# yisol/IDM-VTON

Hardware: NVIDIA H100
Metric: try-on images/sec @768x1024, 30 steps, CFG 2.0 (higher is better)
Workload: dtype fp16

## Files before the change

idm-vton_b200/csrc/gemm.cu:

```cuda
#include "gemm_common.cuh"
#include "host.h"
#include "wgmma.cuh"

namespace vton {

enum : int { KIND_F16 = 0, KIND_F16IN_F32OUT = 1, KIND_TF32 = 2, KIND_E4M3 = 3 };

template <int BN, int STAGES>
struct SmemLayout {
  static constexpr int B_BYTES = BN * 128;
  static constexpr int STAGE_BYTES = A_BYTES + B_BYTES;
  static constexpr int BAR_OFFSET = STAGES * STAGE_BYTES;
  static constexpr int TOTAL = BAR_OFFSET + 256 + 1024;
};

constexpr int GEMM_THREADS = 384;
constexpr int GEMM_PRODUCER_REGS = 40;
constexpr int GEMM_CONSUMER_REGS = 232;

template <int BN>
constexpr int E4M3_SUB = BN == 256 ? 64 : (BN == 192 ? 96 : BN);

template <int BN, int STAGES, bool GEGLU, bool SC, int KIND>
__global__ void __launch_bounds__(GEMM_THREADS, 1)
gemm_conv_kernel(const __grid_constant__ CUtensorMap tmA, const __grid_constant__ CUtensorMap tmB,
                 const __grid_constant__ CUtensorMap tmS0, const __grid_constant__ CUtensorMap tmS1,
                 const __grid_constant__ CUtensorMap tmBs, const GemmParams p) {
  using L = SmemLayout<BN, STAGES>;
  constexpr int KBK = KIND == KIND_TF32 ? 32 : (KIND == KIND_E4M3 ? 128 : 64);
  constexpr bool F16_EPI = KIND == KIND_F16 || KIND == KIND_E4M3;
  extern __shared__ uint8_t smem_raw[];
  const uint32_t smem_base = (smem_u32(smem_raw) + 1023u) & ~1023u;
  const uint32_t bar_base = smem_base + L::BAR_OFFSET;
  auto full_bar = [&](int s) { return bar_base + 8u * s; };
  auto empty_bar = [&](int s) { return bar_base + 8u * (STAGES + s); };

  const int warp = threadIdx.x >> 5;
  const int lane = threadIdx.x & 31;
  const int total_slabs = p.slabs_main + (SC ? p.slabs_sc : 0);

  if (warp == 8 && lane == 0) {
    tma_prefetch_desc(&tmA);
    tma_prefetch_desc(&tmB);
    if (SC) {
      tma_prefetch_desc(&tmS0);
      tma_prefetch_desc(&tmS1);
      tma_prefetch_desc(&tmBs);
    }
    for (int s = 0; s < STAGES; ++s) {
      mbar_init(full_bar(s), 1);
      mbar_init(empty_bar(s), 2);
    }
    fence_barrier_init();
  }
  pdl_wait();
  __syncthreads();
  pdl_launch_dependents();

  if (warp >= 8) {
    setmaxnreg_dec<GEMM_PRODUCER_REGS>();
    if (warp == 8 && lane == 0) {
      uint32_t it = 0;
      for (int tile = blockIdx.x; tile < p.total_tiles; tile += gridDim.x) {
        const int n0 = (tile % p.n_tiles) * BN;
        const int m_tile = tile / p.n_tiles;
        int b0 = 0, y0 = 0, x0 = 0;
        if (p.conv) {
          x0 = (m_tile % p.tiles_x) * p.bw;
          y0 = ((m_tile / p.tiles_x) % p.tiles_y) * p.bh;
          b0 = (m_tile / (p.tiles_x * p.tiles_y)) * p.bb;
        }
        for (int s = 0; s < total_slabs; ++s, ++it) {
          const int stage = it % STAGES;
          const uint32_t phase = (it / STAGES) & 1;
          mbar_wait(empty_bar(stage), phase ^ 1);
          const uint32_t a_dst = smem_base + stage * L::STAGE_BYTES;
          const uint32_t b_dst = a_dst + A_BYTES;
          mbar_expect_tx(full_bar(stage), L::STAGE_BYTES);
          if (s < p.slabs_main) {
            if (p.conv) {
              const int tap = s / p.cin_slabs;
              const int c0 = (s - tap * p.cin_slabs) * KBK;
              const int dy = tap / 3 - 1, dx = tap % 3 - 1;
              tma_load_4d(a_dst, &tmA, full_bar(stage), c0, x0 * p.stride + dx, y0 * p.stride + dy, b0);
              tma_load_2d(b_dst, &tmB, full_bar(stage), c0, tap * p.cout + n0);
            } else {
              tma_load_2d(a_dst, &tmA, full_bar(stage), s * KBK, m_tile * BM);
              tma_load_2d(b_dst, &tmB, full_bar(stage), s * KBK, n0);
            }
          } else {
            const int ss = s - p.slabs_main;
            if (ss < p.sc_split)
              tma_load_4d(a_dst, &tmS0, full_bar(stage), ss * BK, x0, y0, b0);
            else
              tma_load_4d(a_dst, &tmS1, full_bar(stage), (ss - p.sc_split) * BK, x0, y0, b0);
            tma_load_2d(b_dst, &tmBs, full_bar(stage), ss * BK, n0);
          }
        }
      }
    }
    return;
  }

  setmaxnreg_inc<GEMM_CONSUMER_REGS>();
  const int wg = warp >> 2;
  const int r_local = wg * 64 + ((warp & 3) << 4) + (lane >> 2);
  float acc[BN / 2];
  float acc_sc[BN / 2];
  uint32_t it = 0;
  auto release = [&](uint32_t slab) {
    if ((threadIdx.x & 127) == 0) mbar_arrive(empty_bar(slab % STAGES));
  };
  auto run_slabs = [&](float (&accr)[BN / 2], int s_begin, int s_end) {
    for (int s = s_begin; s < s_end; ++s, ++it) {
      const int stage = it % STAGES;
      mbar_wait(full_bar(stage), (it / STAGES) & 1);
      const uint32_t a_src = smem_base + stage * L::STAGE_BYTES + wg * (64 * 128);
      const uint32_t b_src = smem_base + stage * L::STAGE_BYTES + A_BYTES;
      wgmma_fence();
#pragma unroll
      for (int k = 0; k < 4; ++k) {
        const uint64_t da = make_gmma_desc_sw128(a_src + k * 32, 0, 1024);
        const uint64_t db = make_gmma_desc_sw128(b_src + k * 32, 0, 1024);
        const int scale_d = (s > s_begin || k > 0) ? 1 : 0;
        if constexpr (KIND == KIND_TF32) {
          WgmmaTF32SS<BN>::mma(accr, da, db, scale_d);
        } else {
          WgmmaF16SS<BN, 0>::mma(accr, da, db, scale_d);
        }
      }
      wgmma_commit();
      wgmma_wait<1>();
      if (s > 0) release(it - 1);
    }
  };
  auto run_slabs_promoted = [&](float (&accr)[BN / 2], int s_begin, int s_end) {
    constexpr int SUB = E4M3_SUB<BN>;
    for (int s = s_begin; s < s_end; ++s, ++it) {
      const int stage = it % STAGES;
      mbar_wait(full_bar(stage), (it / STAGES) & 1);
      const uint32_t a_src = smem_base + stage * L::STAGE_BYTES + wg * (64 * 128);
      const uint32_t b_src = smem_base + stage * L::STAGE_BYTES + A_BYTES;
#pragma unroll
      for (int sub = 0; sub < BN / SUB; ++sub) {
        float part[SUB / 2];
        wgmma_fence();
#pragma unroll
        for (int k = 0; k < 4; ++k) {
          const uint64_t da = make_gmma_desc_sw128(a_src + k * 32, 0, 1024);
          const uint64_t db = make_gmma_desc_sw128(b_src + sub * SUB * 128 + k * 32, 0, 1024);
          WgmmaE4M3SS<SUB>::mma(part, da, db, k > 0 ? 1 : 0);
        }
        wgmma_commit();
        wgmma_wait<0>();
        fence_regs(part);
#pragma unroll
        for (int j = 0; j < SUB / 2; ++j) accr[sub * (SUB / 2) + j] = s > s_begin ? accr[sub * (SUB / 2) + j] + part[j] : part[j];
      }
      release(it);
    }
  };
  for (int tile = blockIdx.x; tile < p.total_tiles; tile += gridDim.x) {
    EpilogueF16<BN, GEGLU, SC, KIND == KIND_E4M3> epi;
    if constexpr (F16_EPI) epi.begin(p, tile / p.n_tiles, tile % p.n_tiles, r_local);
    if constexpr (KIND == KIND_E4M3) {
      run_slabs_promoted(acc, 0, p.slabs_main);
    } else {
      run_slabs(acc, 0, p.slabs_main);
      if constexpr (SC) run_slabs(acc_sc, p.slabs_main, total_slabs);
      wgmma_wait<0>();
      fence_regs(acc);
      if (SC) fence_regs(acc_sc);
      release(it - 1);
    }
    if constexpr (F16_EPI) {
      epi.finish(p, acc, acc_sc);
    } else {
      epilogue_f32<BN>(p, tile / p.n_tiles, tile % p.n_tiles, r_local, acc);
    }
  }
}

template <int BN, int STAGES, bool GEGLU, bool SC, int KIND>
static int launch_variant(const CUtensorMap& tmA, const CUtensorMap& tmB, const CUtensorMap& tmS0,
                          const CUtensorMap& tmS1, const CUtensorMap& tmBs, const GemmParams& p, cudaStream_t stream) {
  using L = SmemLayout<BN, STAGES>;
  static_assert(L::TOTAL <= 227 * 1024, "shared memory budget");
  auto kern = gemm_conv_kernel<BN, STAGES, GEGLU, SC, KIND>;
  static bool configured = false;
  if (!configured) {
    VTON_CUDA(cudaFuncSetAttribute(kern, cudaFuncAttributeMaxDynamicSharedMemorySize, L::TOTAL));
    configured = true;
  }
  const int grid = p.total_tiles < num_sms() ? p.total_tiles : num_sms();
  VTON_CUDA(launch_kernel(kern, dim3(grid), dim3(GEMM_THREADS), L::TOTAL, stream, tmA, tmB, tmS0, tmS1, tmBs, p));
  count_launch();
  return kOk;
}

void set_auto_v2(int) {}
void set_cluster4(int) {}

static int pick_bn(int N, int m_tiles, bool geglu, bool has_shortcut, int force_bn) {
  if (force_bn >= 2000) force_bn -= 2000;
  else if (force_bn >= 1000) force_bn -= 1000;
  auto usable = [&](int bn) {
    if (geglu && ((bn != 256 && bn != 128) || N % bn != 0)) return false;
    if (has_shortcut && bn > 128) return false;
    return true;
  };
  if (force_bn) {
    const bool known = force_bn == 64 || force_bn == 128 || force_bn == 160 || force_bn == 192 || force_bn == 256;
    return known && usable(force_bn) ? force_bn : 0;
  }
  const int sms = num_sms();
  const int cands[5] = {256, 192, 160, 128, 64};
  double best = 1e300;
  int best_bn = 0;
  for (int bn : cands) {
    if (!usable(bn)) continue;
    if (bn != 128 && N % bn != 0 && !(bn == 64 && N < 64)) continue;
    const long long tiles = static_cast<long long>(m_tiles) * cdiv(N, bn);
    const long long waves = (tiles + sms - 1) / sms;
    const double cost = static_cast<double>(waves) * (bn + 64);
    if (cost < best * 0.999) {
      best = cost;
      best_bn = bn;
    }
  }
  return best_bn ? best_bn : 128;
}

template <int KIND>
static int dispatch(int bn, bool geglu, const CUtensorMap& tmA, const CUtensorMap& tmB, const CUtensorMap& tmS0,
                    const CUtensorMap& tmS1, const CUtensorMap& tmBs, GemmParams& p, int m_tiles,
                    cudaStream_t stream) {
  p.n_tiles = cdiv(p.N, bn);
  p.total_tiles = m_tiles * p.n_tiles;
  if (geglu) {
    if (bn == 128) return launch_variant<128, 6, true, false, KIND>(tmA, tmB, tmS0, tmS1, tmBs, p, stream);
    if (bn == 256) return launch_variant<256, 4, true, false, KIND>(tmA, tmB, tmS0, tmS1, tmBs, p, stream);
    set_last_error("GEGLU epilogue supports BN 128/256 only (got %d)", bn);
    return kErrUnsupported;
  }
  if constexpr (KIND == KIND_F16) {
    if (p.slabs_sc) {
      if (bn == 64) return launch_variant<64, 8, false, true, KIND_F16>(tmA, tmB, tmS0, tmS1, tmBs, p, stream);
      if (bn == 128) return launch_variant<128, 6, false, true, KIND_F16>(tmA, tmB, tmS0, tmS1, tmBs, p, stream);
      set_last_error("shortcut epilogue supports BN 64/128 only (got %d)", bn);
      return kErrUnsupported;
    }
  }
  switch (bn) {
    case 64: return launch_variant<64, 8, false, false, KIND>(tmA, tmB, tmS0, tmS1, tmBs, p, stream);
    case 128: return launch_variant<128, 6, false, false, KIND>(tmA, tmB, tmS0, tmS1, tmBs, p, stream);
    case 160: return launch_variant<160, 5, false, false, KIND>(tmA, tmB, tmS0, tmS1, tmBs, p, stream);
    case 192: return launch_variant<192, 4, false, false, KIND>(tmA, tmB, tmS0, tmS1, tmBs, p, stream);
    case 256: return launch_variant<256, 4, false, false, KIND>(tmA, tmB, tmS0, tmS1, tmBs, p, stream);
  }
  set_last_error("unsupported BN %d", bn);
  return kErrUnsupported;
}

int gemm_f16_impl(const void* A, long long lda, const void* W, long long ldw, void* out, long long ldo, int M, int N,
                  int K, const void* bias, const void* residual, long long ldr, const void* rowvec, long long ld_rowvec,
                  int rows_per_sample, int flags, int force_bn, cudaStream_t stream) {
  const int geglu = flags & 1;
  VTON_CHECK_ARG(M > 0 && N > 0 && K > 0, "gemm: empty problem M=%d N=%d K=%d", M, N, K);
  VTON_CHECK_ARG(K % 64 == 0, "gemm: K=%d must be a multiple of 64", K);
  VTON_CHECK_ARG(N % 8 == 0 && lda % 8 == 0 && ldw % 8 == 0 && ldo % 8 == 0, "gemm: N/lda/ldw/ldo must be multiples of 8");
  VTON_CHECK_ARG(!geglu || (N % 16 == 0 && !residual && !rowvec), "gemm: bad GEGLU configuration");
  VTON_CHECK_ARG(aligned_to(out, 16) && aligned_to(bias, 16) && aligned_to(residual, 16) && aligned_to(rowvec, 16),
                 "gemm: out/bias/residual/rowvec must be 16-byte aligned");
  VTON_CHECK_ARG((!residual || ldr % 8 == 0) && (!rowvec || ld_rowvec % 8 == 0),
                 "gemm: ldr=%lld / ld_rowvec=%lld must be multiples of 8", ldr, ld_rowvec);
  const int bn = pick_bn(N, cdiv(M, BM), geglu != 0, false, force_bn);
  VTON_CHECK_ARG(bn != 0, "gemm: tile width force_bn=%d unsupported for this problem (N=%d, geglu=%d)", force_bn, N, geglu);
  VTON_CHECK_ARG(!geglu || N % bn == 0, "gemm: GEGLU needs N %% BN == 0 (N=%d, BN=%d)", N, bn);
  CUtensorMap tmA, tmB;
  {
    uint64_t dims[2] = {static_cast<uint64_t>(K), static_cast<uint64_t>(M)};
    uint64_t strides[1] = {static_cast<uint64_t>(lda) * 2};
    uint32_t box[2] = {64, 128};
    if (int e = encode_tmap_f16(&tmA, A, 2, dims, strides, box)) return e;
  }
  {
    uint64_t dims[2] = {static_cast<uint64_t>(K), static_cast<uint64_t>(N)};
    uint64_t strides[1] = {static_cast<uint64_t>(ldw) * 2};
    uint32_t box[2] = {64, static_cast<uint32_t>(bn)};
    if (int e = encode_tmap_f16(&tmB, W, 2, dims, strides, box)) return e;
  }
  GemmParams p{};
  p.out = static_cast<__half*>(out);
  p.ld_out = static_cast<int>(ldo);
  p.M = M;
  p.N = N;
  p.bias = static_cast<const __half*>(bias);
  p.residual = static_cast<const __half*>(residual);
  p.ld_res = static_cast<int>(ldr);
  p.rowvec = static_cast<const __half*>(rowvec);
  p.ld_rowvec = static_cast<int>(ld_rowvec);
  p.rows_per_sample = rows_per_sample;
  p.slabs_main = K / 64;
  p.act_gelu = (flags & 4) ? 2 : ((flags & 2) ? 1 : 0);
  return dispatch<KIND_F16>(bn, geglu != 0, tmA, tmB, tmA, tmA, tmB, p, cdiv(M, BM), stream);
}

int gemm_e4m3_impl(const void* A, long long lda, const void* a_scale, const void* W, long long ldw, const void* w_scale,
                   void* out, long long ldo, int M, int N, int K, const void* bias, const void* residual, long long ldr,
                   int flags, int force_bn, cudaStream_t stream) {
  const int geglu = flags & 1;
  VTON_CHECK_ARG(M > 0 && N > 0 && K > 0, "gemm_e4m3: empty problem M=%d N=%d K=%d", M, N, K);
  VTON_CHECK_ARG(K % 128 == 0, "gemm_e4m3: K=%d must be a multiple of 128", K);
  VTON_CHECK_ARG((flags & ~1) == 0, "gemm_e4m3: flags=%d unsupported (only GEGLU = 1)", flags);
  VTON_CHECK_ARG(A && W && out && a_scale && w_scale, "gemm_e4m3: A, W, out, a_scale and w_scale must not be null");
  VTON_CHECK_ARG(lda % 16 == 0 && ldw % 16 == 0, "gemm_e4m3: lda=%lld / ldw=%lld must be multiples of 16 bytes", lda, ldw);
  VTON_CHECK_ARG(N % 8 == 0 && ldo % 8 == 0, "gemm_e4m3: N/ldo must be multiples of 8");
  VTON_CHECK_ARG(!geglu || (N % 16 == 0 && !residual), "gemm_e4m3: bad GEGLU configuration");
  VTON_CHECK_ARG(aligned_to(A, 16) && aligned_to(W, 16) && aligned_to(out, 16) && aligned_to(bias, 16) &&
                     aligned_to(residual, 16) && aligned_to(a_scale, 4) && aligned_to(w_scale, 8),
                 "gemm_e4m3: A/W/out/bias/residual must be 16-byte aligned, a_scale 4-byte, w_scale 8-byte");
  VTON_CHECK_ARG(!residual || ldr % 8 == 0, "gemm_e4m3: ldr=%lld must be a multiple of 8", ldr);
  const int bn = pick_bn(N, cdiv(M, BM), geglu != 0, false, force_bn);
  VTON_CHECK_ARG(bn != 0, "gemm_e4m3: tile width force_bn=%d unsupported for this problem (N=%d, geglu=%d)", force_bn, N,
                 geglu);
  VTON_CHECK_ARG(!geglu || N % bn == 0, "gemm_e4m3: GEGLU needs N %% BN == 0 (N=%d, BN=%d)", N, bn);
  CUtensorMap tmA, tmB;
  {
    uint64_t dims[2] = {static_cast<uint64_t>(K), static_cast<uint64_t>(M)};
    uint64_t strides[1] = {static_cast<uint64_t>(lda)};
    uint32_t box[2] = {128, 128};
    if (int e = encode_tmap_u8(&tmA, A, 2, dims, strides, box)) return e;
  }
  {
    uint64_t dims[2] = {static_cast<uint64_t>(K), static_cast<uint64_t>(N)};
    uint64_t strides[1] = {static_cast<uint64_t>(ldw)};
    uint32_t box[2] = {128, static_cast<uint32_t>(bn)};
    if (int e = encode_tmap_u8(&tmB, W, 2, dims, strides, box)) return e;
  }
  GemmParams p{};
  p.out = static_cast<__half*>(out);
  p.ld_out = static_cast<int>(ldo);
  p.M = M;
  p.N = N;
  p.bias = static_cast<const __half*>(bias);
  p.residual = static_cast<const __half*>(residual);
  p.ld_res = static_cast<int>(ldr);
  p.slabs_main = K / 128;
  p.a_scale = static_cast<const float*>(a_scale);
  p.w_scale = static_cast<const float*>(w_scale);
  return dispatch<KIND_E4M3>(bn, geglu != 0, tmA, tmB, tmA, tmA, tmB, p, cdiv(M, BM), stream);
}

static void pick_box(int B, int H, int W, int* bw, int* bh, int* bb) {
  int w = 1;
  while (w < 128 && W % (w * 2) == 0) w *= 2;
  int h = 1;
  while (w * h < 128 && h * 2 <= H) h *= 2;
  *bw = w;
  *bh = h;
  *bb = 128 / (w * h);
  (void)B;
}

static int encode_nhwc(CUtensorMap* tm, const void* base, int B, int H, int W, int C, int ldc, int bw, int bh, int bb,
                       int pixel_step = 1) {
  uint64_t dims[4] = {static_cast<uint64_t>(C), static_cast<uint64_t>(W), static_cast<uint64_t>(H),
                      static_cast<uint64_t>(B)};
  uint64_t strides[3] = {static_cast<uint64_t>(ldc) * 2, static_cast<uint64_t>(W) * ldc * 2,
                         static_cast<uint64_t>(H) * W * ldc * 2};
  uint32_t box[4] = {64, static_cast<uint32_t>(bw * pixel_step), static_cast<uint32_t>(bh * pixel_step),
                     static_cast<uint32_t>(bb)};
  uint32_t estr[4] = {1, static_cast<uint32_t>(pixel_step), static_cast<uint32_t>(pixel_step), 1};
  return encode_tmap_f16(tm, base, 4, dims, strides, box, pixel_step > 1 ? estr : nullptr);
}

int conv3x3_impl(const void* x, long long ldx, int B, int Hin, int Win, int Cin, const void* w, int Cout, const void* bias,
                 const void* temb, long long ld_temb, const void* sc0, int C0, const void* sc1, int C1, const void* w_sc,
                 const void* bias_sc, const void* residual, long long ldr, void* out, long long ldo, int force_bn,
                 int stride, cudaStream_t stream) {
  VTON_CHECK_ARG(B > 0 && Hin > 0 && Win > 0, "conv3x3: empty input");
  VTON_CHECK_ARG(stride == 1 || stride == 2, "conv3x3: stride %d unsupported", stride);
  VTON_CHECK_ARG(stride == 1 || (!w_sc && !residual), "conv3x3: stride 2 has no shortcut / residual form");
  const int H = (Hin - 1) / stride + 1, W = (Win - 1) / stride + 1;
  VTON_CHECK_ARG(Cin % 64 == 0, "conv3x3: Cin=%d must be a multiple of 64 (pad channels)", Cin);
  VTON_CHECK_ARG(Cout % 8 == 0 && ldo % 8 == 0 && ldx % 8 == 0, "conv3x3: Cout/ldo/ldx must be multiples of 8");
  VTON_CHECK_ARG(C0 % 64 == 0 && C1 % 64 == 0, "conv3x3: shortcut source channels must be multiples of 64");
  VTON_CHECK_ARG(!(w_sc && residual), "conv3x3: shortcut conv and identity residual are exclusive");
  VTON_CHECK_ARG(aligned_to(out, 16) && aligned_to(bias, 16) && aligned_to(temb, 16) && aligned_to(bias_sc, 16) &&
                     aligned_to(residual, 16),
                 "conv3x3: out/bias/temb/bias_sc/residual must be 16-byte aligned");
  VTON_CHECK_ARG((!residual || ldr % 8 == 0) && (!temb || ld_temb % 8 == 0),
                 "conv3x3: ldr=%lld / ld_temb=%lld must be multiples of 8", ldr, ld_temb);
  int bw, bh, bb;
  pick_box(B, H, W, &bw, &bh, &bb);
  const int m_tiles_est = (W / bw) * cdiv(H, bh) * cdiv(B, bb);
  const int bn = pick_bn(Cout, m_tiles_est, false, w_sc != nullptr, force_bn);
  VTON_CHECK_ARG(bn != 0, "conv3x3: tile width force_bn=%d unsupported (a fused shortcut takes 64 or 128)", force_bn);
  CUtensorMap tmA, tmB, tmS0, tmS1, tmBs;
  VTON_CHECK_ARG(stride == 1 || (bw * 2 <= 256 && bh * 2 <= 256), "conv3x3: stride-2 box too large");
  if (int e = encode_nhwc(&tmA, x, B, Hin, Win, Cin, static_cast<int>(ldx), bw, bh, bb, stride)) return e;
  {
    uint64_t dims[2] = {static_cast<uint64_t>(Cin), static_cast<uint64_t>(9) * Cout};
    uint64_t strides[1] = {static_cast<uint64_t>(Cin) * 2};
    uint32_t box[2] = {64, static_cast<uint32_t>(bn)};
    if (int e = encode_tmap_f16(&tmB, w, 2, dims, strides, box)) return e;
  }
  tmS0 = tmA;
  tmS1 = tmA;
  tmBs = tmB;
  GemmParams p{};
  if (w_sc) {
    VTON_CHECK_ARG(sc0 && C0 > 0, "conv3x3: shortcut needs a source");
    if (int e = encode_nhwc(&tmS0, sc0, B, H, W, C0, C0, bw, bh, bb)) return e;
    if (sc1 && C1 > 0) {
      if (int e = encode_nhwc(&tmS1, sc1, B, H, W, C1, C1, bw, bh, bb)) return e;
    }
    const int Csc = C0 + (sc1 ? C1 : 0);
    uint64_t dims[2] = {static_cast<uint64_t>(Csc), static_cast<uint64_t>(Cout)};
    uint64_t strides[1] = {static_cast<uint64_t>(Csc) * 2};
    uint32_t box[2] = {64, static_cast<uint32_t>(bn)};
    if (int e = encode_tmap_f16(&tmBs, w_sc, 2, dims, strides, box)) return e;
    p.slabs_sc = Csc / 64;
    p.sc_split = C0 / 64;
  }
  p.out = static_cast<__half*>(out);
  p.ld_out = static_cast<int>(ldo);
  p.M = B * H * W;
  p.N = Cout;
  p.bias = static_cast<const __half*>(bias);
  p.bias_sc = static_cast<const __half*>(bias_sc);
  p.residual = static_cast<const __half*>(residual);
  p.ld_res = static_cast<int>(ldr);
  p.rowvec = static_cast<const __half*>(temb);
  p.ld_rowvec = static_cast<int>(ld_temb);
  p.slabs_main = 9 * (Cin / 64);
  p.conv = 1;
  p.stride = stride;
  p.H = H;
  p.W = W;
  p.B = B;
  p.bw = bw;
  p.bh = bh;
  p.bb = bb;
  p.tiles_x = W / bw;
  p.tiles_y = cdiv(H, bh);
  p.cin_slabs = Cin / 64;
  p.cout = Cout;
  const int m_tiles = p.tiles_x * p.tiles_y * cdiv(B, bb);
  return dispatch<KIND_F16>(bn, false, tmA, tmB, tmS0, tmS1, tmBs, p, m_tiles, stream);
}

int conv3x3_f32_impl(const void* x, int B, int H, int W, int Cin, const void* w, int Cout, const void* bias,
                     const void* residual, void* out, int in_fp16, cudaStream_t stream) {
  VTON_CHECK_ARG(B > 0 && H > 0 && W > 0, "conv3x3_f32: empty input");
  VTON_CHECK_ARG(Cin % 32 == 0 && Cout % 32 == 0 && Cout >= 64, "conv3x3_f32: Cin=%d / Cout=%d must be multiples of 32 (Cout >= 64)", Cin, Cout);
  VTON_CHECK_ARG(!in_fp16 || Cin % 64 == 0, "conv3x3_f32: fp16 operands need Cin=%d to be a multiple of 64", Cin);
  VTON_CHECK_ARG(x && w && out, "conv3x3_f32: null pointer");
  const int esz = in_fp16 ? 2 : 4;
  const int bk = in_fp16 ? 64 : 32;
  int bw, bh, bb;
  pick_box(B, H, W, &bw, &bh, &bb);
  VTON_CHECK_ARG(bw * bh * bb == 128 && bw >= 8, "conv3x3_f32: W=%d H=%d cannot be tiled into 128-pixel boxes", W, H);
  const int m_tiles = (W / bw) * cdiv(H, bh) * cdiv(B, bb);
  const int bn = pick_bn(Cout, m_tiles, false, false, Cout % 256 == 0 ? 256 : 128);
  CUtensorMap tmA, tmB;
  {
    uint64_t dims[4] = {static_cast<uint64_t>(Cin), static_cast<uint64_t>(W), static_cast<uint64_t>(H), static_cast<uint64_t>(B)};
    uint64_t strides[3] = {static_cast<uint64_t>(Cin) * esz, static_cast<uint64_t>(W) * Cin * esz,
                           static_cast<uint64_t>(H) * W * Cin * esz};
    uint32_t box[4] = {static_cast<uint32_t>(bk), static_cast<uint32_t>(bw), static_cast<uint32_t>(bh), static_cast<uint32_t>(bb)};
    if (int e = in_fp16 ? encode_tmap_f16(&tmA, x, 4, dims, strides, box) : encode_tmap_f32(&tmA, x, 4, dims, strides, box)) return e;
  }
  {
    uint64_t dims[2] = {static_cast<uint64_t>(Cin), static_cast<uint64_t>(9) * Cout};
    uint64_t strides[1] = {static_cast<uint64_t>(Cin) * esz};
    uint32_t box[2] = {static_cast<uint32_t>(bk), static_cast<uint32_t>(bn)};
    if (int e = in_fp16 ? encode_tmap_f16(&tmB, w, 2, dims, strides, box) : encode_tmap_f32(&tmB, w, 2, dims, strides, box)) return e;
  }
  GemmParams p{};
  p.out_f32 = static_cast<float*>(out);
  p.bias_f32 = static_cast<const float*>(bias);
  p.res_f32 = static_cast<const float*>(residual);
  p.M = B * H * W;
  p.N = Cout;
  p.slabs_main = 9 * (Cin / bk);
  p.conv = 1;
  p.stride = 1;
  p.H = H;
  p.W = W;
  p.B = B;
  p.bw = bw;
  p.bh = bh;
  p.bb = bb;
  p.tiles_x = W / bw;
  p.tiles_y = cdiv(H, bh);
  p.cin_slabs = Cin / bk;
  p.cout = Cout;
  p.n_tiles = cdiv(Cout, bn);
  p.total_tiles = m_tiles * p.n_tiles;
  if (in_fp16) {
    if (bn == 256) return launch_variant<256, 4, false, false, KIND_F16IN_F32OUT>(tmA, tmB, tmA, tmA, tmB, p, stream);
    return launch_variant<128, 6, false, false, KIND_F16IN_F32OUT>(tmA, tmB, tmA, tmA, tmB, p, stream);
  }
  if (bn == 256) return launch_variant<256, 4, false, false, KIND_TF32>(tmA, tmB, tmA, tmA, tmB, p, stream);
  return launch_variant<128, 6, false, false, KIND_TF32>(tmA, tmB, tmA, tmA, tmB, p, stream);
}

}
```

idm-vton_b200/csrc/gemm_common.cuh:

```cuda
#pragma once
#include "common.cuh"

namespace vton {

struct GemmParams {
  __half* out;
  int ld_out;
  int M, N;
  const __half* bias;
  const __half* bias_sc;
  const __half* residual;
  int ld_res;
  const __half* rowvec;
  int ld_rowvec;
  int rows_per_sample;
  int slabs_main;
  int slabs_sc;
  int sc_split;
  int conv;
  int H, W, B;
  int bw, bh, bb;
  int tiles_x, tiles_y;
  int cin_slabs;
  int cout;
  int n_tiles;
  int total_tiles;
  int act_gelu;
  int stride;
  float* out_f32;
  const float* bias_f32;
  const float* res_f32;
  const float* a_scale;
  const float* w_scale;
};

constexpr int BM = 128;
constexpr int BK = 64;
constexpr int A_BYTES = BM * BK * 2;

__device__ __forceinline__ void map_row(const GemmParams& p, int m_tile, int r_local, long long* out_row, int* sample) {
  *out_row = -1;
  if (p.conv) {
    const int tx = m_tile % p.tiles_x;
    const int ty = (m_tile / p.tiles_x) % p.tiles_y;
    const int tb = m_tile / (p.tiles_x * p.tiles_y);
    const int lx = r_local % p.bw;
    const int ly = (r_local / p.bw) % p.bh;
    const int lb = r_local / (p.bw * p.bh);
    const int b = tb * p.bb + lb, y = ty * p.bh + ly, x = tx * p.bw + lx;
    if (b < p.B && y < p.H && x < p.W) *out_row = (static_cast<long long>(b) * p.H + y) * p.W + x;
    *sample = b;
  } else {
    const int m = m_tile * BM + r_local;
    if (m < p.M) *out_row = m;
    *sample = p.rows_per_sample > 0 ? m / p.rows_per_sample : 0;
  }
}

__device__ __forceinline__ float gelu_erf_fast(float x) {
  const float ax = fabsf(x) * 0.70710678118654752f;
  const float t = __fdividef(1.0f, fmaf(0.3275911f, ax, 1.0f));
  float poly = fmaf(t, 1.061405429f, -1.453152027f);
  poly = fmaf(poly, t, 1.421413741f);
  poly = fmaf(poly, t, -0.284496736f);
  poly = fmaf(poly, t, 0.254829592f);
  poly *= t;
  float e;
  const float arg = -ax * ax * 1.4426950408889634f;
  asm("ex2.approx.ftz.f32 %0, %1;" : "=f"(e) : "f"(arg));
  const float erf_abs = fmaf(-poly, e, 1.0f);
  const float erf_v = copysignf(erf_abs, x);
  return 0.5f * x * (1.0f + erf_v);
}

__device__ __forceinline__ void quad_transpose(uint32_t (&w)[4], int q) {
  {
    const bool odd = (q & 1) != 0;
    const uint32_t s0 = __shfl_xor_sync(0xffffffffu, odd ? w[0] : w[1], 1);
    const uint32_t s1 = __shfl_xor_sync(0xffffffffu, odd ? w[2] : w[3], 1);
    if (odd) w[0] = s0, w[2] = s1;
    else w[1] = s0, w[3] = s1;
  }
  {
    const bool hi = (q & 2) != 0;
    const uint32_t s0 = __shfl_xor_sync(0xffffffffu, hi ? w[0] : w[2], 2);
    const uint32_t s1 = __shfl_xor_sync(0xffffffffu, hi ? w[1] : w[3], 2);
    if (hi) w[0] = s0, w[1] = s1;
    else w[2] = s0, w[3] = s1;
  }
}

__device__ __forceinline__ float2 ldg_h2(const __half* src) {
  return unpack_h2(__ldg(reinterpret_cast<const uint32_t*>(src)));
}

template <int BN, bool GEGLU, bool SC, bool SCALED = false>
struct EpilogueF16 {
  static constexpr int OUT_COLS = GEGLU ? BN / 2 : BN;
  static constexpr int CHUNKS = OUT_COLS / 32;
  static constexpr bool HAS_RES = !GEGLU && !SC;
  static constexpr int RES_AHEAD = (!HAS_RES || SCALED) ? 1 : (CHUNKS < 4 ? CHUNKS : 4);

  int q, n0, out_n0, out_N;
  long long out_row[2];
  int sample[2];
  uint32_t bias[BN / 8];
  uint32_t bias_sc[SC ? BN / 8 : 1];
  uint4 res[2][RES_AHEAD];
  float a_scale[SCALED ? 2 : 1];

  __device__ __forceinline__ int own_col(int c) const { return out_n0 + (4 * c + q) * 8; }

  __device__ __forceinline__ void load_res(const GemmParams& p, int c) {
#pragma unroll
    for (int h = 0; h < 2; ++h) {
      uint4 u = make_uint4(0u, 0u, 0u, 0u);
      if (p.residual && out_row[h] >= 0 && own_col(c) < out_N)
        u = *reinterpret_cast<const uint4*>(p.residual + out_row[h] * p.ld_res + own_col(c));
      res[h][c % RES_AHEAD] = u;
    }
  }

  __device__ __forceinline__ void begin(const GemmParams& p, int m_tile, int n_tile, int r_local) {
    q = threadIdx.x & 3;
    n0 = n_tile * BN;
    out_n0 = GEGLU ? n_tile * (BN / 2) : n0;
    out_N = GEGLU ? p.N / 2 : p.N;
#pragma unroll
    for (int h = 0; h < 2; ++h) map_row(p, m_tile, r_local + 8 * h, &out_row[h], &sample[h]);
    if constexpr (SCALED) {
#pragma unroll
      for (int h = 0; h < 2; ++h) a_scale[h] = out_row[h] >= 0 ? __ldg(p.a_scale + out_row[h]) : 0.0f;
    }
#pragma unroll
    for (int i = 0; i < BN / 8; ++i) {
      const bool ok = n0 + i * 8 < p.N;
      bias[i] = (p.bias && ok) ? __ldg(reinterpret_cast<const uint32_t*>(p.bias + n0 + i * 8 + 2 * q)) : 0u;
      if (SC) bias_sc[i] = (p.bias_sc && ok) ? __ldg(reinterpret_cast<const uint32_t*>(p.bias_sc + n0 + i * 8 + 2 * q)) : 0u;
    }
    if (HAS_RES) {
#pragma unroll
      for (int c = 0; c < RES_AHEAD; ++c) load_res(p, c);
    }
  }

  __device__ __forceinline__ void finish(const GemmParams& p, const float (&acc)[BN / 2], const float (&acc_sc)[BN / 2]) {
    const __half* rowvec_row[2];
#pragma unroll
    for (int h = 0; h < 2; ++h)
      rowvec_row[h] = (p.rowvec && out_row[h] >= 0) ? p.rowvec + static_cast<long long>(sample[h]) * p.ld_rowvec : nullptr;
#pragma unroll
    for (int c = 0; c < CHUNKS; ++c) {
      if (out_n0 + c * 32 >= out_N) break;
#pragma unroll
      for (int h = 0; h < 2; ++h) {
        uint32_t w[4];
#pragma unroll
        for (int g = 0; g < 4; ++g) {
          const int i = 4 * c + g;
          const bool col_ok = out_n0 + i * 8 < out_N;
          float v0 = acc[4 * i + 2 * h], v1 = acc[4 * i + 2 * h + 1];
          float2 w_scale[GEGLU ? 2 : 1];
          if constexpr (SCALED) {
#pragma unroll
            for (int e = 0; e < (GEGLU ? 2 : 1); ++e) {
              const int col = n0 + (i + e * (BN / 16)) * 8 + 2 * q;
              w_scale[e] = col < p.N ? __ldg(reinterpret_cast<const float2*>(p.w_scale + col)) : make_float2(0.f, 0.f);
            }
            v0 = __fmul_rn(__fmul_rn(v0, a_scale[h]), w_scale[0].x);
            v1 = __fmul_rn(__fmul_rn(v1, a_scale[h]), w_scale[0].y);
          }
          if (GEGLU) {
            float g0 = acc[4 * (i + BN / 16) + 2 * h], g1 = acc[4 * (i + BN / 16) + 2 * h + 1];
            if constexpr (SCALED) {
              g0 = __fmul_rn(__fmul_rn(g0, a_scale[h]), w_scale[GEGLU ? 1 : 0].x);
              g1 = __fmul_rn(__fmul_rn(g1, a_scale[h]), w_scale[GEGLU ? 1 : 0].y);
            }
            if (p.bias && col_ok) {
              const float2 b = unpack_h2(bias[i]), bg = unpack_h2(bias[i + BN / 16]);
              v0 += b.x, v1 += b.y, g0 += bg.x, g1 += bg.y;
            }
            v0 = round_h(v0) * round_h(gelu_erf_fast(round_h(g0)));
            v1 = round_h(v1) * round_h(gelu_erf_fast(round_h(g1)));
          } else {
            if (p.bias && col_ok) {
              const float2 b = unpack_h2(bias[i]);
              v0 += b.x, v1 += b.y;
            }
            if (p.act_gelu) {
              const float x0 = round_h(v0), x1 = round_h(v1);
              v0 = p.act_gelu == 2 ? __fdividef(x0, 1.0f + __expf(-1.702f * x0)) : gelu_erf_fast(x0);
              v1 = p.act_gelu == 2 ? __fdividef(x1, 1.0f + __expf(-1.702f * x1)) : gelu_erf_fast(x1);
            }
            if (rowvec_row[h] != nullptr && col_ok) {
              const float2 t = ldg_h2(rowvec_row[h] + n0 + i * 8 + 2 * q);
              v0 = round_h(v0) + t.x, v1 = round_h(v1) + t.y;
            }
            if (SC) {
              float s0 = acc_sc[4 * i + 2 * h], s1 = acc_sc[4 * i + 2 * h + 1];
              if (p.bias_sc && col_ok) {
                const float2 b = unpack_h2(bias_sc[i]);
                s0 += b.x, s1 += b.y;
              }
              v0 = round_h(s0) + round_h(v0), v1 = round_h(s1) + round_h(v1);
            }
          }
          w[g] = pack_h2(v0, v1);
        }
        quad_transpose(w, q);
        if (out_row[h] < 0 || own_col(c) >= out_N) continue;
        if (HAS_RES && p.residual) {
          const uint4 u = res[h][c % RES_AHEAD];
          const uint32_t r[4] = {u.x, u.y, u.z, u.w};
#pragma unroll
          for (int j = 0; j < 4; ++j) {
            const float2 a = unpack_h2(w[j]), d = unpack_h2(r[j]);
            w[j] = pack_h2(a.x + d.x, a.y + d.y);
          }
        }
        *reinterpret_cast<uint4*>(p.out + out_row[h] * p.ld_out + own_col(c)) = make_uint4(w[0], w[1], w[2], w[3]);
      }
      if (HAS_RES && c + RES_AHEAD < CHUNKS) load_res(p, c + RES_AHEAD);
    }
  }
};

template <int BN>
__device__ __forceinline__ void epilogue_f32(const GemmParams& p, int m_tile, int n_tile, int r_local,
                                             const float (&acc)[BN / 2]) {
  const int q = threadIdx.x & 3;
  const int n0 = n_tile * BN;
  long long out_row[2];
#pragma unroll
  for (int h = 0; h < 2; ++h) {
    int sample;
    map_row(p, m_tile, r_local + 8 * h, &out_row[h], &sample);
  }
#pragma unroll
  for (int i = 0; i < BN / 8; ++i) {
    if (n0 + i * 8 >= p.N) break;
    const int ncol = n0 + i * 8 + 2 * q;
    float2 b = make_float2(0.0f, 0.0f);
    if (p.bias_f32 != nullptr) b = __ldg(reinterpret_cast<const float2*>(p.bias_f32 + ncol));
#pragma unroll
    for (int h = 0; h < 2; ++h) {
      if (out_row[h] < 0) continue;
      float2 v = make_float2(acc[4 * i + 2 * h], acc[4 * i + 2 * h + 1]);
      if (p.bias_f32 != nullptr) v.x += b.x, v.y += b.y;
      if (p.res_f32 != nullptr) {
        const float2 r = __ldg(reinterpret_cast<const float2*>(p.res_f32 + out_row[h] * p.N + ncol));
        v.x += r.x, v.y += r.y;
      }
      *reinterpret_cast<float2*>(p.out_f32 + out_row[h] * p.N + ncol) = v;
    }
  }
}

}
```

Measured before the change: 0.8340.

## Stage GEMM epilogue through shared memory with dedicated store warps

Consumer warpgroups now write finished fp16 tiles into a shared-memory staging buffer instead of storing directly to global memory. Three idle producer-side warps prefetch residual rows with bulk async copies into that buffer and then perform the global stores, synchronised through new mbarriers, so stores overlap the next tile's mainloop. It also specialises the epilogue on activation and rowvec flags, rebalances register limits, and cuts BN=256 stages from 4 to 3 to fit the staging buffer. This adds synchronisation, and the single staging buffer can stall consumers until the store warps finish.

```diff
diff --git a/idm-vton_b200/csrc/gemm.cu b/idm-vton_b200/csrc/gemm.cu
--- a/idm-vton_b200/csrc/gemm.cu
+++ b/idm-vton_b200/csrc/gemm.cu
@@ -6,17 +6,22 @@
 
 enum : int { KIND_F16 = 0, KIND_F16IN_F32OUT = 1, KIND_TF32 = 2, KIND_E4M3 = 3 };
 
-template <int BN, int STAGES>
+constexpr bool f16_out(int kind) { return kind == KIND_F16 || kind == KIND_E4M3; }
+
+template <int BN, int STAGES, bool GEGLU, int KIND>
 struct SmemLayout {
   static constexpr int B_BYTES = BN * 128;
   static constexpr int STAGE_BYTES = A_BYTES + B_BYTES;
-  static constexpr int BAR_OFFSET = STAGES * STAGE_BYTES;
-  static constexpr int TOTAL = BAR_OFFSET + 256 + 1024;
+  static constexpr int STAGING_OFFSET = STAGES * STAGE_BYTES;
+  static constexpr int STAGING_BYTES = f16_out(KIND) ? StagingTile<BN, GEGLU>::BYTES : 0;
+  static constexpr int BAR_OFFSET = STAGING_OFFSET + STAGING_BYTES;
+  static constexpr int ROWS_OFFSET = BAR_OFFSET + 256;
+  static constexpr int TOTAL = ROWS_OFFSET + (f16_out(KIND) ? 2 * BM * 4 : 0) + 1024;
 };
 
 constexpr int GEMM_THREADS = 384;
-constexpr int GEMM_PRODUCER_REGS = 40;
-constexpr int GEMM_CONSUMER_REGS = 232;
+constexpr int GEMM_PRODUCER_REGS = 56;
+constexpr int GEMM_CONSUMER_REGS = 224;
 
 template <int BN>
 constexpr int E4M3_SUB = BN == 256 ? 64 : (BN == 192 ? 96 : BN);
@@ -26,20 +31,23 @@
 gemm_conv_kernel(const __grid_constant__ CUtensorMap tmA, const __grid_constant__ CUtensorMap tmB,
                  const __grid_constant__ CUtensorMap tmS0, const __grid_constant__ CUtensorMap tmS1,
                  const __grid_constant__ CUtensorMap tmBs, const GemmParams p) {
-  using L = SmemLayout<BN, STAGES>;
+  using L = SmemLayout<BN, STAGES, GEGLU, KIND>;
   constexpr int KBK = KIND == KIND_TF32 ? 32 : (KIND == KIND_E4M3 ? 128 : 64);
-  constexpr bool F16_EPI = KIND == KIND_F16 || KIND == KIND_E4M3;
+  constexpr bool F16_EPI = f16_out(KIND);
   extern __shared__ uint8_t smem_raw[];
   const uint32_t smem_base = (smem_u32(smem_raw) + 1023u) & ~1023u;
   const uint32_t bar_base = smem_base + L::BAR_OFFSET;
   auto full_bar = [&](int s) { return bar_base + 8u * s; };
   auto empty_bar = [&](int s) { return bar_base + 8u * (STAGES + s); };
+  const uint32_t staged_bar = bar_base + 8u * (2 * STAGES);
+  const uint32_t ready_bar = bar_base + 8u * (2 * STAGES + 1);
+  const uint32_t staging = smem_base + L::STAGING_OFFSET;
+  auto staging_ptr = [&]() { return smem_raw + (smem_base - smem_u32(smem_raw)) + L::STAGING_OFFSET; };
+  auto row_table = [&]() { return reinterpret_cast<int*>(smem_raw + (smem_base - smem_u32(smem_raw)) + L::ROWS_OFFSET); };
 
   const int warp = threadIdx.x >> 5;
-  const int lane = threadIdx.x & 31;
-  const int total_slabs = p.slabs_main + (SC ? p.slabs_sc : 0);
-
-  if (warp == 8 && lane == 0) {
+
+  if (threadIdx.x == 8 * 32) {
     tma_prefetch_desc(&tmA);
     tma_prefetch_desc(&tmB);
     if (SC) {
@@ -51,6 +59,10 @@
       mbar_init(full_bar(s), 1);
       mbar_init(empty_bar(s), 2);
     }
+    if (F16_EPI) {
+      mbar_init(staged_bar, 256);
+      mbar_init(ready_bar, EpilogueStore<BN, GEGLU>::THREADS);
+    }
     fence_barrier_init();
   }
   pdl_wait();
@@ -59,7 +71,8 @@
 
   if (warp >= 8) {
     setmaxnreg_dec<GEMM_PRODUCER_REGS>();
-    if (warp == 8 && lane == 0) {
+    if (threadIdx.x == 8 * 32) {
+      const int total_slabs = p.slabs_main + (SC ? p.slabs_sc : 0);
       uint32_t it = 0;
       for (int tile = blockIdx.x; tile < p.total_tiles; tile += gridDim.x) {
         const int n0 = (tile % p.n_tiles) * BN;
@@ -98,12 +111,15 @@
           }
         }
       }
+    } else if (F16_EPI && warp > 8) {
+      EpilogueStore<BN, GEGLU>::run(p, staging, staging_ptr(), row_table(), staged_bar, ready_bar, threadIdx.x - 9 * 32);
     }
     return;
   }
 
   setmaxnreg_inc<GEMM_CONSUMER_REGS>();
   const int wg = warp >> 2;
+  const int lane = threadIdx.x & 31;
   const int r_local = wg * 64 + ((warp & 3) << 4) + (lane >> 2);
   float acc[BN / 2];
   float acc_sc[BN / 2];
@@ -167,14 +183,20 @@
       run_slabs_promoted(acc, 0, p.slabs_main);
     } else {
       run_slabs(acc, 0, p.slabs_main);
-      if constexpr (SC) run_slabs(acc_sc, p.slabs_main, total_slabs);
+      if constexpr (SC) run_slabs(acc_sc, p.slabs_main, p.slabs_main + p.slabs_sc);
       wgmma_wait<0>();
       fence_regs(acc);
       if (SC) fence_regs(acc_sc);
       release(it - 1);
     }
     if constexpr (F16_EPI) {
-      epi.finish(p, acc, acc_sc);
+      mbar_wait(ready_bar, ((tile - blockIdx.x) / gridDim.x) & 1);
+      if (!GEGLU && p.act_gelu) epi.template stage<true, true>(p, acc, acc_sc, r_local, staging);
+      else if (!GEGLU && p.rowvec) epi.template stage<false, true>(p, acc, acc_sc, r_local, staging);
+      else epi.template stage<false, false>(p, acc, acc_sc, r_local, staging);
+      mbar_arrive(staged_bar);
+      if (tile + static_cast<int>(gridDim.x) >= p.total_tiles)
+        EpilogueStore<BN, GEGLU>::help_store_last(p, tile, staging_ptr(), row_table(), staged_bar, threadIdx.x);
     } else {
       epilogue_f32<BN>(p, tile / p.n_tiles, tile % p.n_tiles, r_local, acc);
     }
@@ -184,7 +206,7 @@
 template <int BN, int STAGES, bool GEGLU, bool SC, int KIND>
 static int launch_variant(const CUtensorMap& tmA, const CUtensorMap& tmB, const CUtensorMap& tmS0,
                           const CUtensorMap& tmS1, const CUtensorMap& tmBs, const GemmParams& p, cudaStream_t stream) {
-  using L = SmemLayout<BN, STAGES>;
+  using L = SmemLayout<BN, STAGES, GEGLU, KIND>;
   static_assert(L::TOTAL <= 227 * 1024, "shared memory budget");
   auto kern = gemm_conv_kernel<BN, STAGES, GEGLU, SC, KIND>;
   static bool configured = false;
@@ -256,7 +278,7 @@
     case 128: return launch_variant<128, 6, false, false, KIND>(tmA, tmB, tmS0, tmS1, tmBs, p, stream);
     case 160: return launch_variant<160, 5, false, false, KIND>(tmA, tmB, tmS0, tmS1, tmBs, p, stream);
     case 192: return launch_variant<192, 4, false, false, KIND>(tmA, tmB, tmS0, tmS1, tmBs, p, stream);
-    case 256: return launch_variant<256, 4, false, false, KIND>(tmA, tmB, tmS0, tmS1, tmBs, p, stream);
+    case 256: return launch_variant<256, 3, false, false, KIND>(tmA, tmB, tmS0, tmS1, tmBs, p, stream);
   }
   set_last_error("unsupported BN %d", bn);
   return kErrUnsupported;
diff --git a/idm-vton_b200/csrc/gemm_common.cuh b/idm-vton_b200/csrc/gemm_common.cuh
--- a/idm-vton_b200/csrc/gemm_common.cuh
+++ b/idm-vton_b200/csrc/gemm_common.cuh
@@ -94,32 +94,42 @@
   return unpack_h2(__ldg(reinterpret_cast<const uint32_t*>(src)));
 }
 
+__device__ __forceinline__ void st_shared_v4(uint32_t addr, uint32_t a, uint32_t b, uint32_t c, uint32_t d) {
+  asm volatile("st.shared.v4.b32 [%0], {%1, %2, %3, %4};" ::"r"(addr), "r"(a), "r"(b), "r"(c), "r"(d) : "memory");
+}
+__device__ __forceinline__ uint4 ld_shared_v4(uint32_t addr) {
+  uint4 v;
+  asm volatile("ld.shared.v4.b32 {%0, %1, %2, %3}, [%4];" : "=r"(v.x), "=r"(v.y), "=r"(v.z), "=r"(v.w) : "r"(addr) : "memory");
+  return v;
+}
+__device__ __forceinline__ void bulk_copy_g2s(uint32_t dst, const void* src, uint32_t bytes, uint32_t bar) {
+  asm volatile("cp.async.bulk.shared::cluster.global.mbarrier::complete_tx::bytes [%0], [%1], %2, [%3];"
+               ::"r"(dst), "l"(reinterpret_cast<uint64_t>(src)), "r"(bytes), "r"(bar) : "memory");
+}
+
+template <int BN, bool GEGLU>
+struct StagingTile {
+  static constexpr int OUT_COLS = GEGLU ? BN / 2 : BN;
+  static constexpr int CHUNKS_PER_ROW = OUT_COLS / 8;
+  static constexpr int BYTES = BM * OUT_COLS * 2;
+  __device__ static __forceinline__ uint32_t offset(int r, int chunk) {
+    return static_cast<uint32_t>(r * CHUNKS_PER_ROW + chunk) * 16u;
+  }
+};
+
 template <int BN, bool GEGLU, bool SC, bool SCALED = false>
 struct EpilogueF16 {
-  static constexpr int OUT_COLS = GEGLU ? BN / 2 : BN;
+  using Staging = StagingTile<BN, GEGLU>;
+  static constexpr int OUT_COLS = Staging::OUT_COLS;
   static constexpr int CHUNKS = OUT_COLS / 32;
   static constexpr bool HAS_RES = !GEGLU && !SC;
-  static constexpr int RES_AHEAD = (!HAS_RES || SCALED) ? 1 : (CHUNKS < 4 ? CHUNKS : 4);
 
   int q, n0, out_n0, out_N;
   long long out_row[2];
   int sample[2];
   uint32_t bias[BN / 8];
   uint32_t bias_sc[SC ? BN / 8 : 1];
-  uint4 res[2][RES_AHEAD];
   float a_scale[SCALED ? 2 : 1];
-
-  __device__ __forceinline__ int own_col(int c) const { return out_n0 + (4 * c + q) * 8; }
-
-  __device__ __forceinline__ void load_res(const GemmParams& p, int c) {
-#pragma unroll
-    for (int h = 0; h < 2; ++h) {
-      uint4 u = make_uint4(0u, 0u, 0u, 0u);
-      if (p.residual && out_row[h] >= 0 && own_col(c) < out_N)
-        u = *reinterpret_cast<const uint4*>(p.residual + out_row[h] * p.ld_res + own_col(c));
-      res[h][c % RES_AHEAD] = u;
-    }
-  }
 
   __device__ __forceinline__ void begin(const GemmParams& p, int m_tile, int n_tile, int r_local) {
     q = threadIdx.x & 3;
@@ -138,17 +148,17 @@
       bias[i] = (p.bias && ok) ? __ldg(reinterpret_cast<const uint32_t*>(p.bias + n0 + i * 8 + 2 * q)) : 0u;
       if (SC) bias_sc[i] = (p.bias_sc && ok) ? __ldg(reinterpret_cast<const uint32_t*>(p.bias_sc + n0 + i * 8 + 2 * q)) : 0u;
     }
-    if (HAS_RES) {
-#pragma unroll
-      for (int c = 0; c < RES_AHEAD; ++c) load_res(p, c);
-    }
-  }
-
-  __device__ __forceinline__ void finish(const GemmParams& p, const float (&acc)[BN / 2], const float (&acc_sc)[BN / 2]) {
+  }
+
+  template <bool ACT, bool ROWVEC>
+  __device__ __forceinline__ void stage(const GemmParams& p, const float (&acc)[BN / 2], const float (&acc_sc)[BN / 2],
+                                        int r_local, uint32_t staging) {
     const __half* rowvec_row[2];
 #pragma unroll
     for (int h = 0; h < 2; ++h)
-      rowvec_row[h] = (p.rowvec && out_row[h] >= 0) ? p.rowvec + static_cast<long long>(sample[h]) * p.ld_rowvec : nullptr;
+      rowvec_row[h] = (ROWVEC && p.rowvec && out_row[h] >= 0)
+                          ? p.rowvec + static_cast<long long>(sample[h]) * p.ld_rowvec
+                          : nullptr;
 #pragma unroll
     for (int c = 0; c < CHUNKS; ++c) {
       if (out_n0 + c * 32 >= out_N) break;
@@ -187,12 +197,12 @@
               const float2 b = unpack_h2(bias[i]);
               v0 += b.x, v1 += b.y;
             }
-            if (p.act_gelu) {
+            if (ACT && p.act_gelu) {
               const float x0 = round_h(v0), x1 = round_h(v1);
               v0 = p.act_gelu == 2 ? __fdividef(x0, 1.0f + __expf(-1.702f * x0)) : gelu_erf_fast(x0);
               v1 = p.act_gelu == 2 ? __fdividef(x1, 1.0f + __expf(-1.702f * x1)) : gelu_erf_fast(x1);
             }
-            if (rowvec_row[h] != nullptr && col_ok) {
+            if (ROWVEC && rowvec_row[h] != nullptr && col_ok) {
               const float2 t = ldg_h2(rowvec_row[h] + n0 + i * 8 + 2 * q);
               v0 = round_h(v0) + t.x, v1 = round_h(v1) + t.y;
             }
@@ -208,9 +218,9 @@
           w[g] = pack_h2(v0, v1);
         }
         quad_transpose(w, q);
-        if (out_row[h] < 0 || own_col(c) >= out_N) continue;
+        const uint32_t slot = staging + Staging::offset(r_local + 8 * h, 4 * c + q);
         if (HAS_RES && p.residual) {
-          const uint4 u = res[h][c % RES_AHEAD];
+          const uint4 u = ld_shared_v4(slot);
           const uint32_t r[4] = {u.x, u.y, u.z, u.w};
 #pragma unroll
           for (int j = 0; j < 4; ++j) {
@@ -218,9 +228,72 @@
             w[j] = pack_h2(a.x + d.x, a.y + d.y);
           }
         }
-        *reinterpret_cast<uint4*>(p.out + out_row[h] * p.ld_out + own_col(c)) = make_uint4(w[0], w[1], w[2], w[3]);
+        st_shared_v4(slot, w[0], w[1], w[2], w[3]);
       }
-      if (HAS_RES && c + RES_AHEAD < CHUNKS) load_res(p, c + RES_AHEAD);
+    }
+  }
+};
+
+template <int BN, bool GEGLU>
+struct EpilogueStore {
+  using Staging = StagingTile<BN, GEGLU>;
+  static constexpr int THREADS = 96;
+  static constexpr int CPR = Staging::CHUNKS_PER_ROW;
+  static constexpr int UNITS = BM * CPR;
+
+  __device__ static __forceinline__ void store(const GemmParams& p, const uint8_t* staging_ptr, const int* rows, int out_n0,
+                                               int out_N, int t, int n) {
+#pragma unroll 4
+    for (int u = t; u < UNITS; u += n) {
+      const int r = u / CPR, chunk = u % CPR;
+      const int row = rows[r];
+      const int col = out_n0 + chunk * 8;
+      if (row >= 0 && col < out_N)
+        *reinterpret_cast<uint4*>(p.out + static_cast<long long>(row) * p.ld_out + col) =
+            *reinterpret_cast<const uint4*>(staging_ptr + Staging::offset(r, chunk));
+    }
+  }
+
+  __device__ static __forceinline__ void help_store_last(const GemmParams& p, int tile, const uint8_t* staging_ptr,
+                                                         const int* row_table, uint32_t staged_bar, int t) {
+    const int j = (tile - blockIdx.x) / gridDim.x;
+    mbar_wait(staged_bar, j & 1);
+    store(p, staging_ptr, row_table + (j & 1) * BM, (tile % p.n_tiles) * Staging::OUT_COLS, GEGLU ? p.N / 2 : p.N,
+          THREADS + t, THREADS + 256);
+  }
+
+  __device__ static __forceinline__ void run(const GemmParams& p, uint32_t staging, const uint8_t* staging_ptr,
+                                             int* row_table, uint32_t staged_bar, uint32_t ready_bar, int e) {
+    const int out_N = GEGLU ? p.N / 2 : p.N;
+    int j = 0;
+    for (int tile = blockIdx.x; tile < p.total_tiles; tile += gridDim.x, ++j) {
+      const int m_tile = tile / p.n_tiles;
+      const int out_n0 = (tile % p.n_tiles) * Staging::OUT_COLS;
+      int* rows = row_table + (j & 1) * BM;
+      for (int r = e; r < BM; r += THREADS) {
+        long long out_row;
+        int sample;
+        map_row(p, m_tile, r, &out_row, &sample);
+        rows[r] = static_cast<int>(out_row);
+      }
+      named_bar_sync(1, THREADS);
+      if (p.residual) {
+        fence_proxy_async_smem();
+        const uint32_t row_bytes = (out_N - out_n0 < Staging::OUT_COLS ? out_N - out_n0 : Staging::OUT_COLS) * 2u;
+        uint32_t bytes = 0;
+        for (int r = e; r < BM; r += THREADS) bytes += rows[r] >= 0 ? row_bytes : 0u;
+        mbar_expect_tx(ready_bar, bytes);
+        for (int r = e; r < BM; r += THREADS) {
+          if (rows[r] >= 0)
+            bulk_copy_g2s(staging + Staging::offset(r, 0), p.residual + static_cast<long long>(rows[r]) * p.ld_res + out_n0,
+                          row_bytes, ready_bar);
+        }
+      } else {
+        mbar_arrive(ready_bar);
+      }
+      mbar_wait(staged_bar, j & 1);
+      const bool last = tile + static_cast<int>(gridDim.x) >= p.total_tiles;
+      store(p, staging_ptr, rows, out_n0, out_N, e, last ? THREADS + 256 : THREADS);
     }
   }
 };
```

New measurement: 0.9219 (median of 6 runs). 1.11x the previous value.
